# jstmn/cppflow

Measured on NVIDIA B200. Metric: waypoint FK+Jac+collision+LM evals/s, higher is better.
Workload: dtype f32

## Files before the change

### cppflow_b200/csrc/collision.cuh

```cuda
#pragma once
#include "robots.cuh"
#include "kinematics.cuh"
#include "geom.cuh"

namespace cppflow {

__host__ __device__ constexpr double csqrt(double x) {
    if (x <= 0.0) return 0.0;
    double r = x > 1.0 ? x : 1.0;
    for (int i = 0; i < 60; ++i) r = 0.5 * (r + x / r);
    return r;
}
template <class M>
__host__ __device__ constexpr float cap_half_length(int c) {
    const double dx = (double)M::cap(c, 3) - (double)M::cap(c, 0);
    const double dy = (double)M::cap(c, 4) - (double)M::cap(c, 1);
    const double dz = (double)M::cap(c, 5) - (double)M::cap(c, 2);
    return (float)(0.5 * csqrt(dx * dx + dy * dy + dz * dz));
}
#define CPPFLOW_CULL_MARGIN 1e-4f
#define CPPFLOW_AXIS_INSIDE_D2 1e-12f

template <class M>
struct SmemLayout {
    static __host__ __device__ constexpr int alias(int c, int e) {
        const int f = M::cap_frame(c);
        const float x = M::cap(c, 3 * e), y = M::cap(c, 3 * e + 1), z = M::cap(c, 3 * e + 2);
        if (f >= 1 && f <= M::NCHAIN && M::jtype(f - 1) == J_REVOLUTE && x == 0.f && y == 0.f && z == 0.f)
            return dof_of_chain<M>(f - 1);
        if (f < M::NCHAIN && M::jtype(f) != J_FIXED && x == M::origin(f, 0) && y == M::origin(f, 1) && z == M::origin(f, 2))
            return dof_of_chain<M>(f);
        return -1;
    }
    static __host__ __device__ constexpr int n_own() {
        int n = 0;
        for (int c = 0; c < M::NCAP; ++c)
            for (int e = 0; e < 2; ++e) n += alias(c, e) < 0 ? 1 : 0;
        return n;
    }
    static constexpr bool ANY_ALIAS = n_own() < 2 * M::NCAP;
    static constexpr int ORIGINS = n_own() * 3;
    static constexpr int AXES = ORIGINS + M::NDOF * 3;
    static constexpr int N_DIST = ANY_ALIAS ? AXES : ORIGINS;
    static constexpr int N_FULL = AXES + M::NDOF * 3;
    static __host__ __device__ constexpr int slot(int c, int e) {
        const int a = alias(c, e);
        if (a >= 0) return ORIGINS + a * 3;
        int n = 0;
        for (int cc = 0; cc < M::NCAP; ++cc)
            for (int ee = 0; ee < 2; ++ee) {
                if (cc == c && ee == e) return n * 3;
                n += alias(cc, ee) < 0 ? 1 : 0;
            }
        return -1;
    }
    static __host__ __device__ constexpr int slots(int c) { return slot(c, 0) | (slot(c, 1) << 16); }
};
static_assert(SmemLayout<Fetch>::N_FULL == 69 && SmemLayout<Fetch>::N_DIST == 45, "Fetch: 13 of 20 endpoints are joint origins");
static_assert(!SmemLayout<Panda>::ANY_ALIAS && SmemLayout<Panda>::N_DIST == 54, "Panda: every endpoint has its own slot");

template <class M>
struct PairTable {
    int a[M::NPAIR];
    int b[M::NPAIR];
    int fa[M::NPAIR];
    int fb[M::NPAIR];
    float rsum[M::NPAIR];
    float reach[M::NPAIR];
};
template <class M>
__host__ __device__ constexpr PairTable<M> make_pair_table() {
    PairTable<M> t{};
    for (int p = 0; p < M::NPAIR; ++p) {
        t.a[p] = pair_cap<M>(p, 0);
        t.b[p] = pair_cap<M>(p, 1);
        t.fa[p] = M::cap_frame(t.a[p]);
        t.fb[p] = M::cap_frame(t.b[p]);
        t.rsum[p] = M::cap(t.a[p], 6) + M::cap(t.b[p], 6);
        t.reach[p] = t.rsum[p] + cap_half_length<M>(t.a[p]) + cap_half_length<M>(t.b[p]) + CPPFLOW_CULL_MARGIN;
    }
    return t;
}
template <class M>
struct CapTable {
    int frame[M::NCAP];
    int slots[M::NCAP];
    float radius[M::NCAP];
    float reach[M::NCAP];
};
template <class M>
__host__ __device__ constexpr CapTable<M> make_cap_table() {
    CapTable<M> t{};
    for (int c = 0; c < M::NCAP; ++c) {
        t.frame[c] = M::cap_frame(c);
        t.slots[c] = SmemLayout<M>::slots(c);
        t.radius[c] = M::cap(c, 6);
        t.reach[c] = M::cap(c, 6) + cap_half_length<M>(c) + CPPFLOW_CULL_MARGIN;
    }
    return t;
}
template <class M>
__constant__ PairTable<M> c_pair_table = make_pair_table<M>();
template <class M>
__constant__ CapTable<M> c_cap_table = make_cap_table<M>();

template <class M, int BLOCK, bool WITH_JOINTS, int D>
__device__ __forceinline__ void store_joint(float* sm, const float* axis, const float* origin) {
#pragma unroll
    for (int r = 0; r < 3; ++r) {
        if constexpr (WITH_JOINTS) sm[(SmemLayout<M>::AXES + D * 3 + r) * BLOCK] = axis[r];
        if constexpr (WITH_JOINTS || SmemLayout<M>::ANY_ALIAS) sm[(SmemLayout<M>::ORIGINS + D * 3 + r) * BLOCK] = origin[r];
    }
}
template <class M, int BLOCK, int C>
__device__ __forceinline__ void store_capsule(float* sm, const float (&P)[3], const float (&Q)[3]) {
#pragma unroll
    for (int r = 0; r < 3; ++r) {
        if constexpr (SmemLayout<M>::alias(C, 0) < 0) sm[(SmemLayout<M>::slot(C, 0) + r) * BLOCK] = P[r];
        if constexpr (SmemLayout<M>::alias(C, 1) < 0) sm[(SmemLayout<M>::slot(C, 1) + r) * BLOCK] = Q[r];
    }
}

template <class M, int BLOCK, bool WITH_JOINTS>
struct CollisionSink {
    float* sm;
    template <int D>
    __device__ __forceinline__ void joint(std::integral_constant<int, D>, const float* axis, const float* origin) {
        store_joint<M, BLOCK, WITH_JOINTS, D>(sm, axis, origin);
    }
    template <int F>
    __device__ __forceinline__ void frame(std::integral_constant<int, F>, const Frame& fr) {
        static_for<M::NCAP>([&](auto Cc) {
            constexpr int c = decltype(Cc)::value;
            if constexpr (M::cap_frame(c) == F) {
                float P[3], Q[3];
                capsule_endpoint<M, c, 0>(fr, P);
                capsule_endpoint<M, c, 1>(fr, Q);
                store_capsule<M, BLOCK, c>(sm, P, Q);
            }
        });
    }
};

template <int BLOCK>
__device__ __forceinline__ void load_capsule(const float* sm, int slots, float (&P)[3], float (&Q)[3]) {
    const int sp = slots & 0xffff, sq = slots >> 16;
#pragma unroll
    for (int r = 0; r < 3; ++r) {
        P[r] = sm[(sp + r) * BLOCK];
        Q[r] = sm[(sq + r) * BLOCK];
    }
}


template <int BLOCK>
__device__ __forceinline__ float capsule_pair_core(const float* sm, int slots_a, int slots_b, float rsum, float (&C2)[3],
                                                   float (&nrm)[3]) {
    float P1[3], Q1[3], P2[3], Q2[3];
    load_capsule<BLOCK>(sm, slots_a, P1, Q1);
    load_capsule<BLOCK>(sm, slots_b, P2, Q2);
    float s, t;
    segseg_closest(P1, Q1, P2, Q2, s, t);
    float diff[3];
#pragma unroll
    for (int r = 0; r < 3; ++r) {
        const float c1 = fmaf(s, Q1[r] - P1[r], P1[r]);
        C2[r] = fmaf(t, Q2[r] - P2[r], P2[r]);
        diff[r] = c1 - C2[r];
    }
    const float d2 = dot3(diff, diff);
    const float dist = sqrtf(d2);
    const float inv = d2 > 1e-24f ? rsqrtf(d2) : 0.f;
#pragma unroll
    for (int r = 0; r < 3; ++r) nrm[r] = diff[r] * inv;
    return dist - rsum;
}

template <class M, int BLOCK>
__device__ __forceinline__ void capsule_pair_gradient_core(const float* sm, int fa, int fb, const float (&C2)[3],
                                                           const float (&nrm)[3], float (&g)[M::NDOF]) {
    static_for<M::NDOF>([&](auto Dd) {
        constexpr int d = decltype(Dd)::value;
        constexpr int ci = chain_of_dof<M>(d);
        float gd = 0.f;
        if (ci >= fa && ci < fb) {
            float a[3], o[3];
#pragma unroll
            for (int r = 0; r < 3; ++r) {
                a[r] = sm[(SmemLayout<M>::AXES + d * 3 + r) * BLOCK];
                o[r] = sm[(SmemLayout<M>::ORIGINS + d * 3 + r) * BLOCK];
            }
            if constexpr (dof_is_prismatic<M>(d)) {
                gd = -dot3(nrm, a);
            } else {
                const float rr[3] = {C2[0] - o[0], C2[1] - o[1], C2[2] - o[2]};
                float v[3];
                cross3(a, rr, v);
                gd = -dot3(nrm, v);
            }
        }
        g[d] = gd;
    });
}

template <int BLOCK>
__device__ __forceinline__ float capsule_cuboid_core(const float (&P)[3], const float (&Q)[3], const float (&A)[3],
                                                     const float (&B)[3], const Obstacles& ob, int o, float radius,
                                                     float (&Cw)[3], float (&nrm)[3]) {
    const float t = segbox_closest(A, B, ob.lo[o], ob.hi[o]);
    float diff[3];
#pragma unroll
    for (int r = 0; r < 3; ++r) {
        const float cb = fmaf(t, B[r] - A[r], A[r]);
        diff[r] = cb - fminf(fmaxf(cb, ob.lo[o][r]), ob.hi[o][r]);
        Cw[r] = fmaf(t, Q[r] - P[r], P[r]);
    }
    const float d2 = dot3(diff, diff);
    const float dist = sqrtf(d2);
    const float inv = d2 > CPPFLOW_AXIS_INSIDE_D2 ? rsqrtf(d2) : 0.f;
    const float nb[3] = {diff[0] * inv, diff[1] * inv, diff[2] * inv};
    if (ob.has_rot[o]) {
#pragma unroll
        for (int r = 0; r < 3; ++r)
            nrm[r] = fmaf(ob.R[o][3 * r + 2], nb[2], fmaf(ob.R[o][3 * r + 1], nb[1], ob.R[o][3 * r] * nb[0]));
    } else {
        nrm[0] = nb[0]; nrm[1] = nb[1]; nrm[2] = nb[2];
    }
    return dist - radius;
}

template <class M, int BLOCK>
__device__ __forceinline__ void capsule_cuboid_gradient_core(const float* sm, int fc, const float (&Cw)[3],
                                                             const float (&nrm)[3], float (&g)[M::NDOF]) {
    static_for<M::NDOF>([&](auto Dd) {
        constexpr int d = decltype(Dd)::value;
        constexpr int ci = chain_of_dof<M>(d);
        float gd = 0.f;
        if (ci < fc) {
            float a[3], o[3];
#pragma unroll
            for (int r = 0; r < 3; ++r) {
                a[r] = sm[(SmemLayout<M>::AXES + d * 3 + r) * BLOCK];
                o[r] = sm[(SmemLayout<M>::ORIGINS + d * 3 + r) * BLOCK];
            }
            if constexpr (dof_is_prismatic<M>(d)) {
                gd = dot3(nrm, a);
            } else {
                const float rr[3] = {Cw[0] - o[0], Cw[1] - o[1], Cw[2] - o[2]};
                float v[3];
                cross3(a, rr, v);
                gd = dot3(nrm, v);
            }
        }
        g[d] = gd;
    });
}

template <class M, int BLOCK>
__device__ __forceinline__ float self_pair_distance(const float* sm, int p, float (&C2)[3], float (&nrm)[3],
                                                    float cull_thr = INFINITY) {
    const int a = c_cap_table<M>.slots[c_pair_table<M>.a[p]], b = c_cap_table<M>.slots[c_pair_table<M>.b[p]];
    {
        float P1[3], Q1[3], P2[3], Q2[3];
        load_capsule<BLOCK>(sm, a, P1, Q1);
        load_capsule<BLOCK>(sm, b, P2, Q2);
        const float mx = (P1[0] + Q1[0]) - (P2[0] + Q2[0]);
        const float my = (P1[1] + Q1[1]) - (P2[1] + Q2[1]);
        const float mz = (P1[2] + Q1[2]) - (P2[2] + Q2[2]);
        const float lim = cull_thr + c_pair_table<M>.reach[p];
        if (0.25f * (mx * mx + my * my + mz * mz) > lim * lim && lim > 0.f) return INFINITY;
    }
    return capsule_pair_core<BLOCK>(sm, a, b, c_pair_table<M>.rsum[p], C2, nrm);
}
template <class M, int BLOCK>
__device__ __forceinline__ void self_pair_gradient(const float* sm, int p, const float (&C2)[3], const float (&nrm)[3],
                                                   float (&g)[M::NDOF]) {
    capsule_pair_gradient_core<M, BLOCK>(sm, c_pair_table<M>.fa[p], c_pair_table<M>.fb[p], C2, nrm, g);
}
template <class M, int BLOCK>
__device__ __forceinline__ float env_capsule_distance(const float* sm, int c, const Obstacles& ob, int o,
                                                      float (&Cw)[3], float (&nrm)[3], float cull_thr = INFINITY) {
    float P[3], Q[3], A[3], B[3];
    load_capsule<BLOCK>(sm, c_cap_table<M>.slots[c], P, Q);
    to_box_frame(ob, o, P, A);
    to_box_frame(ob, o, Q, B);
    {
        float dd = 0.f;
#pragma unroll
        for (int r = 0; r < 3; ++r) {
            const float m = 0.5f * (A[r] + B[r]);
            const float e = m - fminf(fmaxf(m, ob.lo[o][r]), ob.hi[o][r]);
            dd = fmaf(e, e, dd);
        }
        const float lim = cull_thr + c_cap_table<M>.reach[c];
        if (dd > lim * lim && lim > 0.f) return INFINITY;
    }
    return capsule_cuboid_core<BLOCK>(P, Q, A, B, ob, o, c_cap_table<M>.radius[c], Cw, nrm);
}
template <class M, int BLOCK>
__device__ __forceinline__ void env_capsule_gradient(const float* sm, int c, const float (&Cw)[3],
                                                     const float (&nrm)[3], float (&g)[M::NDOF]) {
    capsule_cuboid_gradient_core<M, BLOCK>(sm, c_cap_table<M>.frame[c], Cw, nrm, g);
}



template <class M>
struct CollTables {
    int pair_ab[M::NPAIR];
    float pair_rsum[M::NPAIR];
    int cap_frame[M::NCAP];
    int cap_slots[M::NCAP];
    float cap_radius[M::NCAP];
    Obstacles ob;
};

template <class M>
__device__ __forceinline__ void fill_coll_tables(CollTables<M>& tb, const Obstacles& ob, int tid, int nthreads) {
    for (int p = tid; p < M::NPAIR; p += nthreads) {
        tb.pair_ab[p] = c_pair_table<M>.a[p] | (c_pair_table<M>.b[p] << 8) | (c_pair_table<M>.fa[p] << 16) |
                        (c_pair_table<M>.fb[p] << 24);
        tb.pair_rsum[p] = c_pair_table<M>.rsum[p];
    }
    for (int c = tid; c < M::NCAP; c += nthreads) {
        tb.cap_frame[c] = c_cap_table<M>.frame[c];
        tb.cap_slots[c] = c_cap_table<M>.slots[c];
        tb.cap_radius[c] = c_cap_table<M>.radius[c];
    }
    const int* src = reinterpret_cast<const int*>(&ob);
    int* dst = reinterpret_cast<int*>(&tb.ob);
    for (int k = tid; k < (int)(sizeof(Obstacles) / sizeof(int)); k += nthreads) dst[k] = src[k];
}

template <class M, int BLOCK, bool WITH_JOINTS>
struct MidSink {
    float* sm;
    float mid2[M::NCAP][3];
    template <int D>
    __device__ __forceinline__ void joint(std::integral_constant<int, D>, const float* axis, const float* origin) {
        store_joint<M, BLOCK, WITH_JOINTS, D>(sm, axis, origin);
    }
    template <int F>
    __device__ __forceinline__ void frame(std::integral_constant<int, F>, const Frame& fr) {
        static_for<M::NCAP>([&](auto Cc) {
            constexpr int c = decltype(Cc)::value;
            if constexpr (M::cap_frame(c) == F) {
                float P[3], Q[3];
                capsule_endpoint<M, c, 0>(fr, P);
                capsule_endpoint<M, c, 1>(fr, Q);
                store_capsule<M, BLOCK, c>(sm, P, Q);
#pragma unroll
                for (int r = 0; r < 3; ++r) mid2[c][r] = P[r] + Q[r];
            }
        });
    }
};

template <class M>
__host__ __device__ constexpr float pair_reach(int p) {
    const int a = pair_cap<M>(p, 0), b = pair_cap<M>(p, 1);
    return M::cap(a, 6) + M::cap(b, 6) + cap_half_length<M>(a) + cap_half_length<M>(b) + CPPFLOW_CULL_MARGIN;
}
template <class M>
__host__ __device__ constexpr float cap_reach(int c) {
    return M::cap(c, 6) + cap_half_length<M>(c) + CPPFLOW_CULL_MARGIN;
}

template <class M>
__device__ __forceinline__ unsigned self_cull_mask(const float (&mid2)[M::NCAP][3]) {
    static_assert(M::NPAIR <= 32, "pair mask is 32 bits");
    unsigned mask = 0u;
    static_for<M::NPAIR>([&](auto Pp) {
        constexpr int p = decltype(Pp)::value;
        constexpr int a = pair_cap<M>(p, 0), b = pair_cap<M>(p, 1);
        constexpr float lim = pair_reach<M>(p);
        constexpr float lim2x4 = 4.f * lim * lim;
        const float mx = mid2[a][0] - mid2[b][0], my = mid2[a][1] - mid2[b][1], mz = mid2[a][2] - mid2[b][2];
        const float dd = fmaf(mz, mz, fmaf(my, my, mx * mx));
        mask |= (dd > lim2x4) ? 0u : (1u << p);
    });
    return mask;
}

template <class M>
__host__ __device__ constexpr int n_static_capsules() {
    int first_moving_frame = M::NCHAIN + 1;
    for (int i = M::NCHAIN - 1; i >= 0; --i)
        if (M::jtype(i) != J_FIXED) first_moving_frame = i + 1;
    int n = 0;
    while (n < M::NCAP && M::cap_frame(n) < first_moving_frame) ++n;
    return n;
}

static_assert(n_static_capsules<Fetch>() == 1 && n_static_capsules<FetchArm>() == 2 && n_static_capsules<Panda>() == 1,
              "base link (and the fixed torso of fetch_arm) are the static capsules");

template <bool SAT>
__device__ __forceinline__ float positive_part(float x) {
    if constexpr (SAT) return __saturatef(x);
    else return fmaxf(x, 0.f);
}
template <class M, int FIRST = 0>
__device__ __forceinline__ unsigned env_cull_mask(const float (&mid2)[M::NCAP][3], const Obstacles& ob, int o) {
    unsigned mask = 0u;
    const float t2[3] = {2.f * ob.t[o][0], 2.f * ob.t[o][1], 2.f * ob.t[o][2]};
    const float cb[3] = {ob.lo[o][0] + ob.hi[o][0], ob.lo[o][1] + ob.hi[o][1], ob.lo[o][2] + ob.hi[o][2]};
    const float hb[3] = {ob.hi[o][0] - ob.lo[o][0], ob.hi[o][1] - ob.lo[o][1], ob.hi[o][2] - ob.lo[o][2]};
    if (ob.has_rot[o]) {
        static_for<M::NCAP - FIRST>([&](auto Cc) {
            constexpr int c = decltype(Cc)::value + FIRST;
            constexpr float lim = cap_reach<M>(c);
            constexpr float lim2x4 = 4.f * lim * lim;
            constexpr bool SAT = lim2x4 < 1.f;
            const float v[3] = {mid2[c][0] - t2[0], mid2[c][1] - t2[1], mid2[c][2] - t2[2]};
            float dd = 0.f;
#pragma unroll
            for (int r = 0; r < 3; ++r) {
                const float m = fmaf(ob.R[o][6 + r], v[2], fmaf(ob.R[o][3 + r], v[1], ob.R[o][r] * v[0]));
                const float e = positive_part<SAT>(fabsf(m - cb[r]) - hb[r]);
                dd = fmaf(e, e, dd);
            }
            mask |= (dd > lim2x4) ? 0u : (1u << c);
        });
    } else {
        const float cw[3] = {cb[0] + t2[0], cb[1] + t2[1], cb[2] + t2[2]};
        static_for<M::NCAP - FIRST>([&](auto Cc) {
            constexpr int c = decltype(Cc)::value + FIRST;
            constexpr float lim = cap_reach<M>(c);
            constexpr float lim2x4 = 4.f * lim * lim;
            constexpr bool SAT = lim2x4 < 1.f;
            float dd = 0.f;
#pragma unroll
            for (int r = 0; r < 3; ++r) {
                const float e = positive_part<SAT>(fabsf(mid2[c][r] - cw[r]) - hb[r]);
                dd = fmaf(e, e, dd);
            }
            mask |= (dd > lim2x4) ? 0u : (1u << c);
        });
    }
    return mask;
}

template <class M, int BLOCK>
__device__ __forceinline__ float self_pair_exact(const float* sm, const CollTables<M>& tb, int p, float (&C2)[3],
                                                 float (&nrm)[3]) {
    const int ab = tb.pair_ab[p];
    return capsule_pair_core<BLOCK>(sm, tb.cap_slots[ab & 0xff], tb.cap_slots[(ab >> 8) & 0xff], tb.pair_rsum[p], C2, nrm);
}
template <class M, int BLOCK>
__device__ __forceinline__ void self_pair_gradient_rt(const float* sm, const CollTables<M>& tb, int p,
                                                      const float (&C2)[3], const float (&nrm)[3], float (&g)[M::NDOF]) {
    const int ab = tb.pair_ab[p];
    capsule_pair_gradient_core<M, BLOCK>(sm, (ab >> 16) & 0xff, (ab >> 24) & 0xff, C2, nrm, g);
}
template <class M, int BLOCK>
__device__ __forceinline__ float env_capsule_exact(const float* sm, const CollTables<M>& tb, int c, int o,
                                                   float (&Cw)[3], float (&nrm)[3]) {
    float P[3], Q[3], A[3], B[3];
    load_capsule<BLOCK>(sm, tb.cap_slots[c], P, Q);
    to_box_frame(tb.ob, o, P, A);
    to_box_frame(tb.ob, o, Q, B);
    return capsule_cuboid_core<BLOCK>(P, Q, A, B, tb.ob, o, tb.cap_radius[c], Cw, nrm);
}
template <class M, int BLOCK>
__device__ __forceinline__ void env_capsule_gradient_rt(const float* sm, const CollTables<M>& tb, int c,
                                                        const float (&Cw)[3], const float (&nrm)[3],
                                                        float (&g)[M::NDOF]) {
    capsule_cuboid_gradient_core<M, BLOCK>(sm, tb.cap_frame[c], Cw, nrm, g);
}

}
```

### cppflow_b200/csrc/k_lm_full.cu

```cuda
#include <cstdlib>

#include "common.cuh"
#include "collision.cuh"
#include "linalg.cuh"

namespace cppflow {

constexpr int ABLOCK = 256;

template <int D>
struct BlockLayout {
    static constexpr int NT = D * (D + 1) / 2;
    static constexpr int NW = ((NT + D) + 3) / 4 * 4;
};

struct AssembleParams {
    float lambda;
    float a_pos, a_rot;
    float w2_self, w2_env;
    float gamma2;
    float beta[CPPFLOW_MAX_DOF];
    int use_pose, use_diff, use_virtual, n_virtual, use_self, use_env;
    int prefetch;
};

__device__ __forceinline__ void axpy2(float s, float x0, float x1, float& y0, float& y1) {
    const float2 r = __ffma2_rn(make_float2(s, s), make_float2(x0, x1), make_float2(y0, y1));
    y0 = r.x;
    y1 = r.y;
}

template <class M>
__device__ __forceinline__ void rank1_update(float (&A)[BlockLayout<M::NDOF>::NT], float (&b)[M::NDOF],
                                             const float (&g)[M::NDOF], float w2, float d) {
    constexpr int D = M::NDOF;
    float wg[D];
#pragma unroll
    for (int i = 0; i < D; ++i) wg[i] = w2 * g[i];
#pragma unroll
    for (int i = 0; i + 1 < D; i += 2) axpy2(-d, wg[i], wg[i + 1], b[i], b[i + 1]);
    if constexpr (D % 2 == 1) b[D - 1] = fmaf(-d, wg[D - 1], b[D - 1]);
#pragma unroll
    for (int i = 0; i < D; ++i) {
#pragma unroll
        for (int j = 0; j + 1 <= i; j += 2) axpy2(wg[i], g[j], g[j + 1], A[tri(i, j)], A[tri(i, j + 1)]);
        if (i % 2 == 0) A[tri(i, i)] = fmaf(wg[i], g[i], A[tri(i, i)]);
    }
}

template <int D>
__device__ __forceinline__ void load_row(const float* __restrict__ p, float (&x)[D]) {
    if constexpr (D % 4 == 0) {
#pragma unroll
        for (int d = 0; d < D; d += 4) {
            const float4 v = __ldg(reinterpret_cast<const float4*>(p + d));
            x[d] = v.x; x[d + 1] = v.y; x[d + 2] = v.z; x[d + 3] = v.w;
        }
    } else {
#pragma unroll
        for (int d = 0; d < D; ++d) x[d] = __ldg(p + d);
    }
}

__device__ __forceinline__ float wrap_pi_lm(float d) {
    const float k = floorf(fmaf(d, 0.15915494309189535f, 0.5f));
    return fmaf(k, -6.28318548202514648f, d);
}

struct SolveParams {
    float b_rev, b_pri;
    float pivot_floor;
    int do_clamp;
    unsigned zero;
};

template <class M>
struct BetaSel {
    float b_rev, b_pri, rr, rp, pp;
    __device__ __forceinline__ BetaSel(float b_rev_, float b_pri_)
        : b_rev(b_rev_), b_pri(b_pri_), rr(b_rev_ * b_rev_), rp(b_rev_ * b_pri_), pp(b_pri_ * b_pri_) {}
    template <int d>
    __device__ __forceinline__ float b() const { return dof_is_prismatic<M>(d) ? b_pri : b_rev; }
    template <int i, int j>
    __device__ __forceinline__ float bb() const {
        return (dof_is_prismatic<M>(i) && dof_is_prismatic<M>(j)) ? pp
               : (dof_is_prismatic<M>(i) || dof_is_prismatic<M>(j)) ? rp : rr;
    }
};

#ifdef CPPFLOW_SOLVE_TIMING
__device__ unsigned long long g_solve_cycles[8];
#define PHASE_T(var) const long long var = clock64()
#define PHASE_DECL long long ph_acc[7] = {0, 0, 0, 0, 0, 0, 0}
#define PHASE_ADD(i, a, b) ph_acc[i] += (b) - (a)
#define PHASE_FLUSH if (lane == 0) { for (int i_ = 0; i_ < 7; ++i_) atomicAdd(&g_solve_cycles[i_], (unsigned long long)ph_acc[i_]); }
extern "C" int cppflow_debug_solve_cycles(unsigned long long* h_out, int reset) {
    if (reset) { unsigned long long z[8] = {}; cudaMemcpyToSymbol(g_solve_cycles, z, sizeof(z)); return 0; }
    cudaMemcpyFromSymbol(h_out, g_solve_cycles, sizeof(unsigned long long) * 8);
    return 0;
}
#else
#define PHASE_T(var)
#define PHASE_DECL
#define PHASE_ADD(i, a, b)
#define PHASE_FLUSH
#endif

struct FuseParams {
    int* flags;
    int* ticket;
    int npb;
    const float* q;
    float* x_out;
    SolveParams sp;
};
__device__ __forceinline__ int ld_acquire_gpu(const int* p) {
    int v;
    asm volatile("ld.acquire.gpu.global.s32 %0, [%1];" : "=r"(v) : "l"(p) : "memory");
    return v;
}
__device__ __forceinline__ void st_release_gpu(int* p, int v) {
    asm volatile("st.release.gpu.global.s32 [%0], %1;" ::"l"(p), "r"(v) : "memory");
}

template <class M, bool FUSE>
__global__ void __launch_bounds__(ABLOCK, 2)
lm_assemble_kernel(const float* __restrict__ q, const float* __restrict__ xv, const float* __restrict__ target,
                   int P, int T, const Obstacles ob, const AssembleParams prm, float* __restrict__ ws, const FuseParams fz) {
    constexpr int D = M::NDOF;
    constexpr int NT = BlockLayout<D>::NT;
    constexpr int NW = BlockLayout<D>::NW;
    extern __shared__ float smem[];
    __shared__ CollTables<M> tb;
    fill_coll_tables<M>(tb, ob, threadIdx.x, ABLOCK);
    int t, pbx, f_side = 0, f_k = 0;
    bool f_middle = false;
    if constexpr (FUSE) {
        __shared__ int s_ticket;
        if (threadIdx.x == 0) s_ticket = atomicAdd(fz.ticket, 1);
        __syncthreads();
        const int row = s_ticket / fz.npb;
        pbx = s_ticket - row * fz.npb;
        const int m = T / 2, n1 = T - 1 - m;
        if (row < 2 * n1) { f_k = row >> 1; f_side = row & 1; t = f_side ? T - 1 - f_k : f_k; }
        else if (row < T - 1) { f_k = n1; f_side = 0; t = n1; }
        else { f_middle = true; t = m; }
    } else {
        t = blockIdx.y;
        pbx = blockIdx.x;
    }
    const int pth_raw = pbx * ABLOCK + threadIdx.x;
    const bool live = pth_raw < P;
    const int pth = live ? pth_raw : P - 1;
    const int64_t i = (int64_t)pth * T + t;
    float* sm = smem + threadIdx.x;

    float x[D], dwrap[D], vwrap[D];
    const bool has_prev = t > 0, has_next = t < T - 1;
    const bool in_virtual = prm.use_virtual && (t < prm.n_virtual || t >= T - prm.n_virtual);
    load_row<D>(q + i * D, x);
    if (prm.prefetch > 0 && t + prm.prefetch < T)
        asm volatile("prefetch.global.L2 [%0];" ::"l"(q + (i + prm.prefetch) * D));
    float tg[7];
    if (prm.use_pose) {
#pragma unroll
        for (int k = 0; k < 7; ++k) tg[k] = __ldg(target + (int64_t)t * 7 + k);
    }
    if (prm.use_diff) {
        float xp[D], xn[D];
        load_row<D>(q + (has_prev ? i - 1 : i) * D, xp);
        load_row<D>(q + (has_next ? i + 1 : i) * D, xn);
#pragma unroll
        for (int d = 0; d < D; ++d) dwrap[d] = wrap_pi_lm(xn[d] - x[d]) - wrap_pi_lm(x[d] - xp[d]);
    }
    if (in_virtual && xv) {
        float xvv[D];
        load_row<D>(xv + i * D, xvv);
#pragma unroll
        for (int d = 0; d < D; ++d) vwrap[d] = wrap_pi_lm(x[d] - xvv[d]);
    }
    __syncthreads();

    MidSink<M, ABLOCK, true> sink;
    sink.sm = sm;
    Frame F;
    fk_chain<M>(x, sink, F);

    float A[NT], b[D];
#pragma unroll
    for (int k = 0; k < NT; ++k) A[k] = 0.f;
#pragma unroll
    for (int d = 0; d < D; ++d) b[d] = 0.f;

    if (prm.use_self) {
        unsigned mask = self_cull_mask<M>(sink.mid2);
        while (mask) {
            const int p = __ffs(mask) - 1;
            mask &= mask - 1;
            float C2[3], nrm[3];
            const float d = self_pair_exact<M, ABLOCK>(sm, tb, p, C2, nrm);
            if (d < 0.f) {
                float g[D];
                self_pair_gradient_rt<M, ABLOCK>(sm, tb, p, C2, nrm, g);
                rank1_update<M>(A, b, g, prm.w2_self, d);
            }
        }
    }
    if (prm.use_env) {
        constexpr int OGRP = 64 / M::NCAP;
        for (int o0 = 0; o0 < tb.ob.n; o0 += OGRP) {
            unsigned long long mask = 0ull;
#pragma unroll 1
            for (int oo = 0; oo < OGRP; ++oo)
                if (o0 + oo < tb.ob.n)
                    mask |= (unsigned long long)env_cull_mask<M, n_static_capsules<M>()>(sink.mid2, tb.ob, o0 + oo) << (oo * M::NCAP);
            while (mask) {
                const int bit = __ffsll((long long)mask) - 1;
                mask &= mask - 1;
                const int oo = bit / M::NCAP, c = bit - oo * M::NCAP;
                float Cw[3], nrm[3];
                const float d = env_capsule_exact<M, ABLOCK>(sm, tb, c, o0 + oo, Cw, nrm);
                if (d < 0.f) {
                    float g[D];
                    env_capsule_gradient_rt<M, ABLOCK>(sm, tb, c, Cw, nrm, g);
                    rank1_update<M>(A, b, g, prm.w2_env, d);
                }
            }
        }
    }

    if (prm.use_pose) {
        float e[6];
        pose_error(tg, F, e);
        float J[6][D];
        static_for<D>([&](auto Dd) {
            constexpr int d = decltype(Dd)::value;
            float a[3], o[3];
#pragma unroll
            for (int r = 0; r < 3; ++r) {
                a[r] = sm[(SmemLayout<M>::AXES + d * 3 + r) * ABLOCK];
                o[r] = sm[(SmemLayout<M>::ORIGINS + d * 3 + r) * ABLOCK];
            }
            if constexpr (dof_is_prismatic<M>(d)) {
                J[0][d] = 0.f; J[1][d] = 0.f; J[2][d] = 0.f;
                J[3][d] = a[0] * prm.a_pos; J[4][d] = a[1] * prm.a_pos; J[5][d] = a[2] * prm.a_pos;
            } else {
                const float rr[3] = {F.p[0] - o[0], F.p[1] - o[1], F.p[2] - o[2]};
                float v[3];
                cross3(a, rr, v);
                J[0][d] = a[0] * prm.a_rot; J[1][d] = a[1] * prm.a_rot; J[2][d] = a[2] * prm.a_rot;
                J[3][d] = v[0] * prm.a_pos; J[4][d] = v[1] * prm.a_pos; J[5][d] = v[2] * prm.a_pos;
            }
        });
#pragma unroll
        for (int r = 0; r < 3; ++r) { e[r] *= prm.a_rot; e[r + 3] *= prm.a_pos; }
#pragma unroll
        for (int r = 0; r < 6; ++r) {
#pragma unroll
            for (int c = 0; c + 1 < D; c += 2) axpy2(e[r], J[r][c], J[r][c + 1], b[c], b[c + 1]);
            if constexpr (D % 2 == 1) b[D - 1] = fmaf(e[r], J[r][D - 1], b[D - 1]);
        }
        static_for<D>([&](auto Cc) {
            constexpr int c = decltype(Cc)::value;
            static_for<(c + 2) / 2>([&](auto Hh) {
                constexpr int c2 = 2 * decltype(Hh)::value;
                if constexpr (c2 + 1 <= c) {
                    constexpr int r0 = (dof_is_prismatic<M>(c) || (dof_is_prismatic<M>(c2) && dof_is_prismatic<M>(c2 + 1))) ? 3 : 0;
#pragma unroll
                    for (int r = r0; r < 6; ++r) axpy2(J[r][c], J[r][c2], J[r][c2 + 1], A[tri(c, c2)], A[tri(c, c2 + 1)]);
                } else {
                    constexpr int r0 = dof_is_prismatic<M>(c) ? 3 : 0;
                    float v = A[tri(c, c)];
#pragma unroll
                    for (int r = r0; r < 6; ++r) v = fmaf(J[r][c], J[r][c], v);
                    A[tri(c, c)] = v;
                }
            });
        });
    }

    if (prm.use_diff) {
        const float nt = (has_prev ? 1.f : 0.f) + (has_next ? 1.f : 0.f);
#pragma unroll
        for (int d = 0; d < D; ++d) {
            b[d] = fmaf(prm.beta[d], dwrap[d], b[d]);
            A[tri(d, d)] = fmaf(prm.beta[d], nt, A[tri(d, d)]);
        }
    }
    if (in_virtual) {
#pragma unroll
        for (int d = 0; d < D; ++d) {
            A[tri(d, d)] += prm.gamma2;
            if (xv) b[d] = fmaf(-prm.gamma2, vwrap[d], b[d]);
        }
    }
#pragma unroll
    for (int d = 0; d < D; ++d) A[tri(d, d)] += prm.lambda;

    float4* grp = reinterpret_cast<float4*>(ws) + (int64_t)(pth >> 4) * T * (NW / 4 * 16) + (pth & 15);
    auto block_at = [&](int tt) { return grp + (int64_t)tt * (NW / 4 * 16); };
    auto store_blk = [&](int tt, const float (&S)[NT], const float (&y)[D]) {
        float blk[NW];
#pragma unroll
        for (int k = 0; k < NT; ++k) blk[k] = S[k];
#pragma unroll
        for (int d = 0; d < D; ++d) blk[NT + d] = y[d];
#pragma unroll
        for (int k = NT + D; k < NW; ++k) blk[k] = 0.f;
        float4* out = block_at(tt);
#pragma unroll
        for (int k = 0; k < NW / 4; ++k) out[k * 16] = make_float4(blk[4 * k], blk[4 * k + 1], blk[4 * k + 2], blk[4 * k + 3]);
    };
    if constexpr (!FUSE) {
        if (live) store_blk(t, A, b);
    } else {
        constexpr int NWARP = ABLOCK / 32;
        const int warp = threadIdx.x >> 5, lane = threadIdx.x & 31;
        const BetaSel<M> bs(fz.sp.b_rev, fz.sp.b_pri);
        int* flags_pb = fz.flags + pbx * 2 * NWARP;
        auto wait_for = [&](const int* flag, int need) {
            if (lane == 0) {
                while (ld_acquire_gpu(flag) < need) __nanosleep(64);
            }
            __syncwarp();
        };
        auto load_blk = [&](int tt, float (&v)[NW]) {
            const float4* src = block_at(tt);
#pragma unroll
            for (int k = 0; k < NW / 4; ++k) {
                const float4 f = __ldcg(src + k * 16);
                v[4 * k] = f.x; v[4 * k + 1] = f.y; v[4 * k + 2] = f.z; v[4 * k + 3] = f.w;
            }
        };
        if (!f_middle) {
            int* flag = flags_pb + f_side * NWARP + warp;
            float u[D];
            if (f_k > 0) {
                wait_for(flag, f_k);
                float pb_[NW];
                load_blk(f_side ? t + 1 : t - 1, pb_);
                static_for<D>([&](auto Ii) {
                    constexpr int i = decltype(Ii)::value;
                    u[i] = fmaf(bs.template b<i>(), pb_[NT + i], b[i]);
                    static_for<i + 1>([&](auto Jj) {
                        constexpr int j = decltype(Jj)::value;
                        A[tri(i, j)] = fmaf(bs.template bb<i, j>(), pb_[tri(i, j)], A[tri(i, j)]);
                    });
                });
            } else {
                static_for<D>([&](auto Ii) {
                    constexpr int i = decltype(Ii)::value;
                    u[i] = fmaf(bs.template b<i>(), 0.f, b[i]);
                    static_for<i + 1>([&](auto Jj) {
                        constexpr int j = decltype(Jj)::value;
                        A[tri(i, j)] = fmaf(bs.template bb<i, j>(), 0.f, A[tri(i, j)]);
                    });
                });
            }
            sweep_neg_inverse<D>(A, u, fz.sp.pivot_floor);
            if (live) store_blk(t, A, u);
            __threadfence();
            __syncwarp();
            if (lane == 0) st_release_gpu(flag, f_k + 1);
        } else {
            const int m = t, n0 = m, n1 = T - 1 - m;
            float dx[D];
            float L[NW], Rb[NW];
            if (n0 > 0) { wait_for(flags_pb + warp, n0); load_blk(m - 1, L); }
            else {
#pragma unroll
                for (int k = 0; k < NW; ++k) L[k] = 0.f;
            }
            if (n1 > 0) { wait_for(flags_pb + NWARP + warp, n1); load_blk(m + 1, Rb); }
            else {
#pragma unroll
                for (int k = 0; k < NW; ++k) Rb[k] = 0.f;
            }
            static_for<D>([&](auto Ii) {
                constexpr int i = decltype(Ii)::value;
                dx[i] = fmaf(bs.template b<i>(), L[NT + i] + Rb[NT + i], b[i]);
                static_for<i + 1>([&](auto Jj) {
                    constexpr int j = decltype(Jj)::value;
                    A[tri(i, j)] = fmaf(bs.template bb<i, j>(), L[tri(i, j)] + Rb[tri(i, j)], A[tri(i, j)]);
                });
            });
            sweep_neg_inverse<D>(A, dx, fz.sp.pivot_floor);
            if (live) {
                store_blk(m, A, dx);
                float xn[D];
                load_row<D>(fz.q + i * D, xn);
                static_for<D>([&](auto Dd) {
                    constexpr int d = decltype(Dd)::value;
                    xn[d] += dx[d];
                    if (fz.sp.do_clamp) xn[d] = fminf(fmaxf(xn[d], dof_lower<M>(d)), dof_upper<M>(d));
                });
                float* xo = fz.x_out + i * D;
#pragma unroll
                for (int d = 0; d < D; ++d) xo[d] = xn[d];
            }
        }
    }
}

template <int NW>
__device__ __forceinline__ void load_block(const float* __restrict__ p, float (&v)[NW]) {
    const float4* s = reinterpret_cast<const float4*>(p);
#pragma unroll
    for (int k = 0; k < NW / 4; ++k) {
        const float4 f = s[k];
        v[4 * k] = f.x; v[4 * k + 1] = f.y; v[4 * k + 2] = f.z; v[4 * k + 3] = f.w;
    }
}
template <int NW>
__device__ __forceinline__ void store_block(float* __restrict__ p, const float (&v)[NW]) {
    float4* s = reinterpret_cast<float4*>(p);
#pragma unroll
    for (int k = 0; k < NW / 4; ++k) s[k] = make_float4(v[4 * k], v[4 * k + 1], v[4 * k + 2], v[4 * k + 3]);
}

constexpr int SOLVE_WARPS_DEFAULT = 4;
constexpr int SOLVE_RING_ALONE = 3;
constexpr int SOLVE_RING_OVERLAP = 4;

__device__ __forceinline__ unsigned smem_u32(const void* p) { return (unsigned)__cvta_generic_to_shared(p); }
template <bool CG = false>
__device__ __forceinline__ void cp_async16(void* smem, const void* gmem) {
    if constexpr (CG) asm volatile("cp.async.cg.shared.global [%0], [%1], 16;" ::"r"(smem_u32(smem)), "l"(gmem) : "memory");
    else asm volatile("cp.async.ca.shared.global [%0], [%1], 16;" ::"r"(smem_u32(smem)), "l"(gmem) : "memory");
}
__device__ __forceinline__ void cp_async4(void* smem, const void* gmem) {
    asm volatile("cp.async.ca.shared.global [%0], [%1], 4;" ::"r"(smem_u32(smem)), "l"(gmem) : "memory");
}
__device__ __forceinline__ void cp_async_commit() { asm volatile("cp.async.commit_group;" ::: "memory"); }
template <int N>
__device__ __forceinline__ void cp_async_wait() { asm volatile("cp.async.wait_group %0;" ::"n"(N) : "memory"); }

__device__ __forceinline__ void mbar_init(uint64_t* bar) {
    asm volatile("mbarrier.init.shared::cta.b64 [%0], 1;" ::"r"(smem_u32(bar)) : "memory");
}
__device__ __forceinline__ void mbar_expect_tx(uint64_t* bar, unsigned bytes) {
    asm volatile("mbarrier.arrive.expect_tx.shared::cta.b64 _, [%0], %1;" ::"r"(smem_u32(bar)), "r"(bytes) : "memory");
}
__device__ __forceinline__ void mbar_wait(uint64_t* bar, unsigned parity) {
    asm volatile(
        "{\n"
        ".reg .pred p;\n"
        "WAIT_%=:\n"
        "mbarrier.try_wait.parity.shared::cta.b64 p, [%0], %1;\n"
        "@p bra DONE_%=;\n"
        "bra WAIT_%=;\n"
        "DONE_%=:\n"
        "}\n" ::"r"(smem_u32(bar)), "r"(parity) : "memory");
}
__device__ __forceinline__ void bulk_g2s(void* smem, const void* gmem, unsigned bytes, uint64_t* bar) {
    asm volatile("cp.async.bulk.shared::cluster.global.mbarrier::complete_tx::bytes [%0], [%1], %2, [%3];"
                 ::"r"(smem_u32(smem)), "l"(gmem), "r"(bytes), "r"(smem_u32(bar)) : "memory");
}
template <int D, int SOLVE_RING>
struct SolveSmem {
    static constexpr int NV = BlockLayout<D>::NW / 4;
    static constexpr int BLK_BYTES = NV * 16 * 16;
    static constexpr int SLOT_BYTES = (2 * BLK_BYTES + 64 + 127) / 128 * 128;
    static constexpr int Q_BYTES = ((D + 3) / 4) * 16 * 32;
    static constexpr int OFF_Q = SOLVE_RING * SLOT_BYTES;
    static constexpr int BYTES = (OFF_Q + SOLVE_RING * Q_BYTES + 127) / 128 * 128;
    __device__ static unsigned char* part(unsigned char* slot, int side) { return slot + side * (BLK_BYTES + 64); }
    __device__ static float4* blk(unsigned char* part, int k, int l) { return reinterpret_cast<float4*>(part) + k * 16 + l; }
    __device__ static float* qv(unsigned char* base, int slot, int d, int lane) {
        return reinterpret_cast<float*>(base + OFF_Q + (size_t)slot * Q_BYTES) + ((d >> 2) * 32 + lane) * 4 + (d & 3);
    }
};

__device__ __forceinline__ void mbar_expect_tx_a(unsigned bar, unsigned bytes) {
    asm volatile("mbarrier.arrive.expect_tx.shared::cta.b64 _, [%0], %1;" ::"r"(bar), "r"(bytes) : "memory");
}
__device__ __forceinline__ void mbar_wait_a(unsigned bar, unsigned parity) {
    asm volatile(
        "{\n"
        ".reg .pred p;\n"
        "WAIT_%=:\n"
        "mbarrier.try_wait.parity.shared::cta.b64 p, [%0], %1;\n"
        "@p bra DONE_%=;\n"
        "bra WAIT_%=;\n"
        "DONE_%=:\n"
        "}\n" ::"r"(bar), "r"(parity) : "memory");
}
__device__ __forceinline__ void bulk_g2s_a(unsigned dst, const void* gmem, unsigned bytes, unsigned bar) {
    asm volatile("cp.async.bulk.shared::cluster.global.mbarrier::complete_tx::bytes [%0], [%1], %2, [%3];"
                 ::"r"(dst), "l"(gmem), "r"(bytes), "r"(bar) : "memory");
}
__device__ __forceinline__ void cp_async16_a(unsigned dst, const void* gmem) {
    asm volatile("cp.async.ca.shared.global [%0], [%1], 16;" ::"r"(dst), "l"(gmem) : "memory");
}
__device__ __forceinline__ void cp_async4_a(unsigned dst, const void* gmem) {
    asm volatile("cp.async.ca.shared.global [%0], [%1], 4;" ::"r"(dst), "l"(gmem) : "memory");
}

template <class M, int SOLVE_RING, int SOLVE_WARPS, bool BACK_ONLY = false>
__global__ void __launch_bounds__(32 * SOLVE_WARPS, 512 / (32 * SOLVE_WARPS))
lm_block_solve_kernel(const float* __restrict__ q, int64_t P, int64_t T64, const SolveParams prm, float* __restrict__ ws,
                      float* __restrict__ x_out) {
    constexpr int D = M::NDOF;
    constexpr int NT = BlockLayout<D>::NT;
    constexpr int NW = BlockLayout<D>::NW;
    constexpr int NV = NW / 4;
    using SM = SolveSmem<D, SOLVE_RING>;
    extern __shared__ __align__(128) unsigned char smem_all[];
    const int warp = __shfl_sync(0xffffffffu, (int)(threadIdx.x >> 5), 0), lane = threadIdx.x & 31;
    const int64_t g = (int64_t)blockIdx.x * SOLVE_WARPS + warp;
    __shared__ uint64_t s_bars[SOLVE_WARPS][SOLVE_RING];
    if (lane == 0) {
#pragma unroll
        for (int j = 0; j < SOLVE_RING; ++j) mbar_init(s_bars[warp] + j);
        asm volatile("fence.mbarrier_init.release.cluster;" ::: "memory");
    }
    __syncthreads();
    if (g * 16 >= P) return;
    const int T = (int)T64;
    unsigned char* sm = smem_all + (size_t)warp * SM::BYTES;
    const unsigned sm_a = smem_u32(sm);
    const unsigned bar_a = smem_u32(s_bars[warp]);
    const int side = lane & 1, l = lane >> 1;
    const int64_t p_raw = g * 16 + l;
    const bool active = p_raw < P;
    const int64_t p = active ? p_raw : P - 1;
    unsigned char* wsg = reinterpret_cast<unsigned char*>(ws) + g * T64 * SM::BLK_BYTES;
    const float* qp = q + p * T64 * D;
    float* xp = x_out + p * T64 * D;
    const int m = T / 2;
// ... 886 lines not shown
```

### profiles/sass_histogram.py

```python
import collections
import os
import re
import subprocess
import sys
import tempfile

REPO = os.path.dirname(os.path.dirname(os.path.abspath(__file__)))
LIB = sys.argv[1] if len(sys.argv) > 1 else os.path.join(REPO, "cppflow_b200", "libcppflow_b200.so")
SHOW = ["UBLKCP", "SYNCS", "UCGABAR_ARV", "UCGABAR_WAIT", "REDUX", "SHFL", "FFMA2", "FFMA", "FADD", "FMUL", "FMNMX", "FMNMX3",
        "FSETP", "MUFU", "LDG", "STG", "LDS", "STS", "LDGSTS", "ATOMS", "ATOMG", "MEMBAR", "BAR", "STL", "LDL", "UTCMMA",
        "LDTM", "UTMALDG"]


def demangle(names):
    out = subprocess.run(["cu++filt"] + names, capture_output=True, text=True).stdout.splitlines()
    names = []
    for o in out:
        o = o.replace("void ", "").replace("cppflow::", "").replace("(bool)0", "false").replace("(bool)1", "true")
        o = o.replace("(int)", "")
        names.append(o.split(">(")[0] + ">" if ">(" in o else o.split("(")[0])
    return names


def main():
    tmp = tempfile.mkdtemp()
    subprocess.run(["cuobjdump", "-xelf", "all", os.path.abspath(LIB)], cwd=tmp, capture_output=True)
    res = subprocess.run(["cuobjdump", "--dump-resource-usage", os.path.abspath(LIB)], capture_output=True, text=True).stdout
    regs = {}
    fn = None
    for ln in res.splitlines():
        m = re.search(r"Function (\S+):", ln)
        if m:
            fn = m.group(1)
        m = re.search(r"REG:(\d+) STACK:(\d+) SHARED:(\d+)", ln)
        if m and fn:
            regs[fn] = (int(m.group(1)), int(m.group(2)), int(m.group(3)))
    rows = []
    for f in sorted(os.listdir(tmp)):
        if not f.endswith(".cubin"):
            continue
        txt = subprocess.run(["nvdisasm", "-c", os.path.join(tmp, f)], capture_output=True, text=True).stdout
        cur, ops = None, None
        for ln in txt.splitlines():
            m = re.match(r"\s*\.text\.(\S+):", ln)
            if m:
                cur = m.group(1)
                ops = collections.Counter()
                rows.append((cur, ops))
                continue
            m = re.match(r"\s+/\*[0-9a-f]{4,}\*/\s+(?:@!?U?P\d+\s+)?([A-Z0-9_]+)", ln)
            if m and ops is not None:
                ops[m.group(1)] += 1
    rows = [(n, o) for n, o in rows if sum(o.values()) > 0 and ("FetchTILb0" in n or "cppflow" in n and "Fetch" not in n and "Panda" not in n)]
    names = demangle([n for n, _ in rows])
    print("# SASS opcode histogram per kernel (sm_100a cubins of libcppflow_b200.so; `python profiles/sass_histogram.py`)\n")
    print("Fetch instantiations (`FetchT<false>`) and the robot-independent kernels; counts are static instructions.\n")
    used = [k for k in SHOW if any(o.get(k, 0) for _, o in rows)]
    print("| kernel | instr | regs | stack B | " + " | ".join(used) + " |")
    print("|---|---|---|---|" + "---|" * len(used))
    tot = collections.Counter()
    for (mangled, ops), name in sorted(zip(rows, names), key=lambda t: t[1]):
        r = regs.get(mangled, ("?", "?", "?"))
        print(f"| `{name[:88]}` | {sum(ops.values())} | {r[0]} | {r[1]} | " + " | ".join(str(ops.get(k, 0)) for k in used) + " |")
        tot.update(ops)
    print("\nWhole library (all robots): " + ", ".join(f"{k} {v}" for k, v in tot.most_common(12)))
    absent = [k for k in ("UTCMMA", "LDTM", "UTMALDG") if not tot.get(k)]
    print("\nAbsent, as expected for a path without GEMM-shaped work: " + ", ".join(absent))


if __name__ == "__main__":
    main()
```

Before: 4.743 billion.

## Pair cull tests into f32x2 ops and hoist env cull masks before exact tests

Self-pair and axis-aligned environment cull tests now process two pairs or capsules at once using packed float2 FMA/ADD/MUL intrinsics, which is meant to halve the scalar FP instruction count in the culling prologue. The LM kernel also computes all environment cull masks up front into two 64-bit masks before running the self and env exact-distance loops, rather than interleaving culling and exact tests per obstacle group. The shared axpy2 helper moves into a new header. The hoisting adds live 64-bit mask registers across the self loop, and the packed ops need extra MOVs to pair operands.

```diff
diff --git a/cppflow_b200/csrc/collision.cuh b/cppflow_b200/csrc/collision.cuh
--- a/cppflow_b200/csrc/collision.cuh
+++ b/cppflow_b200/csrc/collision.cuh
@@ -2,6 +2,7 @@
 #include "robots.cuh"
 #include "kinematics.cuh"
 #include "geom.cuh"
+#include "f32x2.cuh"
 
 namespace cppflow {
 
@@ -370,15 +371,27 @@
 __device__ __forceinline__ unsigned self_cull_mask(const float (&mid2)[M::NCAP][3]) {
     static_assert(M::NPAIR <= 32, "pair mask is 32 bits");
     unsigned mask = 0u;
-    static_for<M::NPAIR>([&](auto Pp) {
-        constexpr int p = decltype(Pp)::value;
+    static_for<M::NPAIR / 2>([&](auto Pp) {
+        constexpr int p = 2 * decltype(Pp)::value;
+        constexpr int a0 = pair_cap<M>(p, 0), b0 = pair_cap<M>(p, 1), a1 = pair_cap<M>(p + 1, 0), b1 = pair_cap<M>(p + 1, 1);
+        constexpr float lim0 = pair_reach<M>(p), lim1 = pair_reach<M>(p + 1);
+        constexpr float l0 = 4.f * lim0 * lim0, l1 = 4.f * lim1 * lim1;
+        float2 m[3];
+#pragma unroll
+        for (int r = 0; r < 3; ++r) m[r] = make_float2(mid2[a0][r] - mid2[b0][r], mid2[a1][r] - mid2[b1][r]);
+        const float2 dd = fma2(m[2], m[2], fma2(m[1], m[1], mul2(m[0], m[0])));
+        mask |= (dd.x > l0) ? 0u : (1u << p);
+        mask |= (dd.y > l1) ? 0u : (1u << (p + 1));
+    });
+    if constexpr (M::NPAIR % 2 == 1) {
+        constexpr int p = M::NPAIR - 1;
         constexpr int a = pair_cap<M>(p, 0), b = pair_cap<M>(p, 1);
         constexpr float lim = pair_reach<M>(p);
         constexpr float lim2x4 = 4.f * lim * lim;
         const float mx = mid2[a][0] - mid2[b][0], my = mid2[a][1] - mid2[b][1], mz = mid2[a][2] - mid2[b][2];
         const float dd = fmaf(mz, mz, fmaf(my, my, mx * mx));
         mask |= (dd > lim2x4) ? 0u : (1u << p);
-    });
+    }
     return mask;
 }
 
@@ -424,8 +437,23 @@
         });
     } else {
         const float cw[3] = {cb[0] + t2[0], cb[1] + t2[1], cb[2] + t2[2]};
-        static_for<M::NCAP - FIRST>([&](auto Cc) {
-            constexpr int c = decltype(Cc)::value + FIRST;
+        static_for<(M::NCAP - FIRST) / 2>([&](auto Cc) {
+            constexpr int c = 2 * decltype(Cc)::value + FIRST;
+            constexpr float lim0 = cap_reach<M>(c), lim1 = cap_reach<M>(c + 1);
+            constexpr float l0 = 4.f * lim0 * lim0, l1 = 4.f * lim1 * lim1;
+            float2 dd;
+#pragma unroll
+            for (int r = 0; r < 3; ++r) {
+                const float2 d = sub2(make_float2(mid2[c][r], mid2[c + 1][r]), bcast2(cw[r]));
+                const float2 e = make_float2(positive_part<(l0 < 1.f)>(fabsf(d.x) - hb[r]),
+                                             positive_part<(l1 < 1.f)>(fabsf(d.y) - hb[r]));
+                dd = r == 0 ? mul2(e, e) : fma2(e, e, dd);
+            }
+            mask |= (dd.x > l0) ? 0u : (1u << c);
+            mask |= (dd.y > l1) ? 0u : (1u << (c + 1));
+        });
+        if constexpr ((M::NCAP - FIRST) % 2 == 1) {
+            constexpr int c = M::NCAP - 1;
             constexpr float lim = cap_reach<M>(c);
             constexpr float lim2x4 = 4.f * lim * lim;
             constexpr bool SAT = lim2x4 < 1.f;
@@ -436,7 +464,7 @@
                 dd = fmaf(e, e, dd);
             }
             mask |= (dd > lim2x4) ? 0u : (1u << c);
-        });
+        }
     }
     return mask;
 }
diff --git a/cppflow_b200/csrc/f32x2.cuh b/cppflow_b200/csrc/f32x2.cuh
--- /dev/null
+++ b/cppflow_b200/csrc/f32x2.cuh
@@ -0,0 +1,17 @@
+#pragma once
+#include <cuda_runtime.h>
+
+namespace cppflow {
+
+__device__ __forceinline__ float2 bcast2(float s) { return make_float2(s, s); }
+__device__ __forceinline__ float2 sub2(float2 a, float2 b) { return __fadd2_rn(a, make_float2(-b.x, -b.y)); }
+__device__ __forceinline__ float2 mul2(float2 a, float2 b) { return __fmul2_rn(a, b); }
+__device__ __forceinline__ float2 fma2(float2 a, float2 b, float2 c) { return __ffma2_rn(a, b, c); }
+
+__device__ __forceinline__ void axpy2(float s, float x0, float x1, float& y0, float& y1) {
+    const float2 r = fma2(bcast2(s), make_float2(x0, x1), make_float2(y0, y1));
+    y0 = r.x;
+    y1 = r.y;
+}
+
+}
diff --git a/cppflow_b200/csrc/k_lm_full.cu b/cppflow_b200/csrc/k_lm_full.cu
--- a/cppflow_b200/csrc/k_lm_full.cu
+++ b/cppflow_b200/csrc/k_lm_full.cu
@@ -23,12 +23,6 @@
     int use_pose, use_diff, use_virtual, n_virtual, use_self, use_env;
     int prefetch;
 };
-
-__device__ __forceinline__ void axpy2(float s, float x0, float x1, float& y0, float& y1) {
-    const float2 r = __ffma2_rn(make_float2(s, s), make_float2(x0, x1), make_float2(y0, y1));
-    y0 = r.x;
-    y1 = r.y;
-}
 
 template <class M>
 __device__ __forceinline__ void rank1_update(float (&A)[BlockLayout<M::NDOF>::NT], float (&b)[M::NDOF],
@@ -192,39 +186,43 @@
 #pragma unroll
     for (int d = 0; d < D; ++d) b[d] = 0.f;
 
-    if (prm.use_self) {
-        unsigned mask = self_cull_mask<M>(sink.mid2);
+    constexpr int OGRP = 64 / M::NCAP;
+    static_assert(2 * OGRP >= CPPFLOW_MAX_OBSTACLES, "two survivor masks cover every obstacle");
+    unsigned self_mask = prm.use_self ? self_cull_mask<M>(sink.mid2) : 0u;
+    unsigned long long env_mask0 = 0ull, env_mask1 = 0ull;
+    if (prm.use_env) {
+#pragma unroll 1
+        for (int o = 0; o < tb.ob.n; ++o) {
+            const unsigned long long m = env_cull_mask<M, n_static_capsules<M>()>(sink.mid2, tb.ob, o);
+            if (o < OGRP) env_mask0 |= m << (o * M::NCAP);
+            else env_mask1 |= m << ((o - OGRP) * M::NCAP);
+        }
+    }
+    while (self_mask) {
+        const int p = __ffs(self_mask) - 1;
+        self_mask &= self_mask - 1;
+        float C2[3], nrm[3];
+        const float d = self_pair_exact<M, ABLOCK>(sm, tb, p, C2, nrm);
+        if (d < 0.f) {
+            float g[D];
+            self_pair_gradient_rt<M, ABLOCK>(sm, tb, p, C2, nrm, g);
+            rank1_update<M>(A, b, g, prm.w2_self, d);
+        }
+    }
+#pragma unroll 1
+    for (int grp = 0; grp < 2; ++grp) {
+        unsigned long long mask = grp ? env_mask1 : env_mask0;
+        const int o0 = grp * OGRP;
         while (mask) {
-            const int p = __ffs(mask) - 1;
+            const int bit = __ffsll((long long)mask) - 1;
             mask &= mask - 1;
-            float C2[3], nrm[3];
-            const float d = self_pair_exact<M, ABLOCK>(sm, tb, p, C2, nrm);
+            const int oo = bit / M::NCAP, c = bit - oo * M::NCAP;
+            float Cw[3], nrm[3];
+            const float d = env_capsule_exact<M, ABLOCK>(sm, tb, c, o0 + oo, Cw, nrm);
             if (d < 0.f) {
                 float g[D];
-                self_pair_gradient_rt<M, ABLOCK>(sm, tb, p, C2, nrm, g);
-                rank1_update<M>(A, b, g, prm.w2_self, d);
-            }
-        }
-    }
-    if (prm.use_env) {
-        constexpr int OGRP = 64 / M::NCAP;
-        for (int o0 = 0; o0 < tb.ob.n; o0 += OGRP) {
-            unsigned long long mask = 0ull;
-#pragma unroll 1
-            for (int oo = 0; oo < OGRP; ++oo)
-                if (o0 + oo < tb.ob.n)
-                    mask |= (unsigned long long)env_cull_mask<M, n_static_capsules<M>()>(sink.mid2, tb.ob, o0 + oo) << (oo * M::NCAP);
-            while (mask) {
-                const int bit = __ffsll((long long)mask) - 1;
-                mask &= mask - 1;
-                const int oo = bit / M::NCAP, c = bit - oo * M::NCAP;
-                float Cw[3], nrm[3];
-                const float d = env_capsule_exact<M, ABLOCK>(sm, tb, c, o0 + oo, Cw, nrm);
-                if (d < 0.f) {
-                    float g[D];
-                    env_capsule_gradient_rt<M, ABLOCK>(sm, tb, c, Cw, nrm, g);
-                    rank1_update<M>(A, b, g, prm.w2_env, d);
-                }
+                env_capsule_gradient_rt<M, ABLOCK>(sm, tb, c, Cw, nrm, g);
+                rank1_update<M>(A, b, g, prm.w2_env, d);
             }
         }
     }
diff --git a/profiles/sass_histogram.py b/profiles/sass_histogram.py
--- a/profiles/sass_histogram.py
+++ b/profiles/sass_histogram.py
@@ -7,7 +7,7 @@
 
 REPO = os.path.dirname(os.path.dirname(os.path.abspath(__file__)))
 LIB = sys.argv[1] if len(sys.argv) > 1 else os.path.join(REPO, "cppflow_b200", "libcppflow_b200.so")
-SHOW = ["UBLKCP", "SYNCS", "UCGABAR_ARV", "UCGABAR_WAIT", "REDUX", "SHFL", "FFMA2", "FFMA", "FADD", "FMUL", "FMNMX", "FMNMX3",
+SHOW = ["UBLKCP", "SYNCS", "UCGABAR_ARV", "UCGABAR_WAIT", "REDUX", "SHFL", "FFMA2", "FADD2", "FMUL2", "FFMA", "FADD", "FMUL", "FMNMX", "FMNMX3", "MOV",
         "FSETP", "MUFU", "LDG", "STG", "LDS", "STS", "LDGSTS", "ATOMS", "ATOMG", "MEMBAR", "BAR", "STL", "LDL", "UTCMMA",
         "LDTM", "UTMALDG"]
 
```

Result: no change. 4.806 billion, median of 6 (+1.3%).
